# kuailehaha/liuzhou

Measured on AMD Instinct MI355X. Metric: self-play positions/sec (fixed sims/move), higher is better.
Workload: dtype f16

## Files before the change

### include/liuzhou_hip.h

```cpp
#ifndef LIUZHOU_HIP_H
#define LIUZHOU_HIP_H

#include <stdint.h>

#ifdef __cplusplus
extern "C" {
#endif

#if defined(_WIN32)
#define LZ_API
#else
#define LZ_API __attribute__((visibility("default")))
#endif

typedef enum LzStatus {
    LZ_OK = 0,
    LZ_ERR_ARG = -1,
    LZ_ERR_UNSUPPORTED = -2,
    LZ_ERR_LAUNCH = -3,
    LZ_ERR_ALIGN = -4,
    LZ_ERR_ILLEGAL = -5
} LzStatus;


// ... 359 lines not shown

LZ_API int lz_policy_value_loss_fwd_bwd(const float* log_p1, const float* log_p2, const float* log_pmc,
                                        const float* value_logits, const uint8_t* legal_mask,
                                        const float* policy_target, const float* value_target,
                                        const float* soft_value_target, int64_t batch, float soft_label_alpha,
                                        float anti_draw_penalty, float policy_draw_weight,
                                        const float* policy_weight_sum, float grad_scale, float* terms,
                                        float* grad_log_p1, float* grad_log_p2, float* grad_log_pmc,
                                        float* grad_value_logits, void* stream);


#define LZ_TRAJECTORY_RECORD_BYTES 360
LZ_API int lz_pack_trajectory_rows(const float* state_tensors, const uint8_t* legal_masks,
                                   const float* policy_targets, const float* value_targets,
                                   const float* soft_value_targets, int64_t rows, void* records,
                                   int32_t* not_representable, void* stream);
LZ_API int lz_unpack_trajectory_rows(const void* records, int64_t rows, float* state_tensors, uint8_t* legal_masks,
                                     float* policy_targets, float* value_targets, float* soft_value_targets,
                                     void* stream);


LZ_API int lz_symmetry_tables(int32_t* cells, int32_t* actions, int32_t* inverse, int32_t* compose, int32_t* directions);

LZ_API int lz_symmetry_gather_samples(const float* planes, const uint8_t* masks, const float* policy, int64_t n_src,
                                      const int64_t* idx, const void* sym, int32_t sym_width, float* out_planes,
                                      uint8_t* out_masks, float* out_policy, int64_t m, void* stream);

LZ_API int lz_symmetry_transform_states(const LzStateSoA* in, const void* sym, int32_t sym_width,
                                        const LzStateSoA* out, int64_t batch, void* stream);

LZ_API int lz_symmetry_transform_packed(const int64_t* in , const void* sym, int32_t sym_width,
                                        int64_t* out , int64_t batch, void* stream);

#ifdef __cplusplus
}
#endif
#endif
```

### liuzhou_amd/build.py

```python
from __future__ import annotations

import os
import shutil
import subprocess

PKG = os.path.dirname(os.path.abspath(__file__))
CSRC = os.path.join(PKG, "csrc")
LIB = os.path.join(PKG, "libliuzhou_hip.so")
SOURCES = ("lz_ops.hip", "lz_engine.hip", "lz_net.hip", "lz_net_f32.hip", "lz_train.hip", "lz_search.hip", "lz_symmetry.hip")
HEADERS = ("lz_rules.h", "lz_soa.h", "lz_symmetry.h", "lz_wave.h", "lz_rng.h", "lz_net_dev.h", "lz_tree_dev.h", os.path.join("..", "..", "include", "liuzhou_hip.h"))


def hipcc_path() -> str:
    for cand in (os.environ.get("HIPCC"), "/opt/rocm/bin/hipcc", shutil.which("hipcc")):
        if cand and os.path.exists(cand):
            return cand
    raise RuntimeError("hipcc not found (expected /opt/rocm/bin/hipcc)")


HOST_LIB = os.path.join(PKG, "libliuzhou_host.so")
HOST_SOURCE = os.path.join(CSRC, "lz_host.cpp")
HOST_SOURCES = (HOST_SOURCE, os.path.join(CSRC, "lz_scalar.cpp"),
                os.path.join(CSRC, "lz_symmetry_host.cpp"))


def build_host(force: bool = False, verbose: bool = False) -> str:
    deps = list(HOST_SOURCES) + [os.path.join(CSRC, h) for h in HEADERS] + [os.path.join(PKG, "..", "include", "liuzhou_scalar.h")]
    if not force and os.path.exists(HOST_LIB) and all(
            (not os.path.exists(d)) or os.path.getmtime(d) <= os.path.getmtime(HOST_LIB) for d in deps):
        return HOST_LIB
    cxx = os.environ.get("CXX") or shutil.which("g++") or shutil.which("c++")
    if not cxx:
        raise RuntimeError("no host C++ compiler (g++) found for libliuzhou_host.so")
    cmd = [cxx, "-O2", "-std=c++17", "-ffp-contract=off", "-fPIC", "-shared", "-fvisibility=hidden", "-o", HOST_LIB,
           *HOST_SOURCES]
    if verbose:
        print(" ".join(cmd))
    subprocess.check_call(cmd)
    return HOST_LIB


def needs_build() -> bool:
    if not os.path.exists(LIB):
# ... 76 lines not shown
```

### liuzhou_amd/csrc/lz_engine.hip

```cpp
#include <hip/hip_runtime.h>
#include <hip/amd_detail/amd_hip_unsafe_atomics.h>
#include <math.h>
#include <stdint.h>

#include <mutex>

#include "lz_rng.h"
#include "lz_tree_dev.h"

namespace {

__global__ __launch_bounds__(kBlock) void pack_states_kernel(LzStateSoA s, int64_t B, Packed* __restrict__ out) {
    const int64_t i = (int64_t)blockIdx.x * kBlock + threadIdx.x;
    if (i >= B) return;
    State st;
    st.black = cells_equal(s.board + i * 36, 1);
    st.white = cells_equal(s.board + i * 36, -1);
    st.mb = cells_nonzero(s.marks_black + i * 36);
    st.mw = cells_nonzero(s.marks_white + i * 36);
    st.phase = (int)s.phase[i]; st.player = (int)s.current_player[i];
    st.pm_req = (int)s.pending_marks_required[i]; st.pm_rem = (int)s.pending_marks_remaining[i];
    st.pc_req = (int)s.pending_captures_required[i]; st.pc_rem = (int)s.pending_captures_remaining[i];
    st.forced = (int)s.forced_removals_done[i]; st.move_count = (int)s.move_count[i];
    st.msc = (int)s.moves_since_capture[i];
// ... 1434 lines not shown
    const int64_t rn = next_sims + 1;
    if (rn > d->node_cap) return LZ_ERR_ARG;
    if ((int64_t)d->chunk_cap * (d->edge_chunk - (kMaxChildren - 1)) < (int64_t)d->node_cap * kMaxChildren) return LZ_ERR_ARG;
    const bool big = words > kMarkWordsMax;
    const int wpb = big ? 1 : kWavesPerBlock;
    const size_t lds = (size_t)wpb * (words * (sizeof(uint64_t) + sizeof(int)) + 3 * kWave * sizeof(int));
    if (big) {
        static std::mutex mu;
        static bool configured[64] = {};
        int dev = 0;
        if (hipGetDevice(&dev) != hipSuccess || dev < 0 || dev >= 64) return LZ_ERR_LAUNCH;
        std::lock_guard<std::mutex> lk(mu);
        if (!configured[dev]) {
            const size_t most = (size_t)kMarkWordsBig * (sizeof(uint64_t) + sizeof(int)) + 3 * kWave * sizeof(int);
            if (hipFuncSetAttribute(reinterpret_cast<const void*>(tree_advance_kernel<1>),
                                    hipFuncAttributeMaxDynamicSharedMemorySize, (int)most) != hipSuccess) {
                (void)hipGetLastError();
                return LZ_ERR_LAUNCH;
            }
            configured[dev] = true;
        }
    }
    (void)lz_prof_aux_begin(1, stream);
    if (big)
        hipLaunchKernelGGL(tree_advance_kernel<1>, dim3((unsigned)d->num_games), dim3(kWave), lds, as_stream(stream), make_tree(d),
                           played_action, reset, (int)rn, words, dropped, pruned, g_advance_ticks);
    else
        hipLaunchKernelGGL(tree_advance_kernel<kWavesPerBlock>, dim3(gw(d->num_games)), dim3(kBlock), lds, as_stream(stream),
                           make_tree(d), played_action, reset, (int)rn, words, dropped, pruned, g_advance_ticks);
    (void)lz_prof_aux_end(1, stream, d->num_games);
    return st();
}

extern "C++" template <bool CAP, bool FORCED, bool GUMBEL = false>
static int tree_search_launch(const LzTreeDesc* d, const Tree& t, const CapArrays& cap, const ForcedArgs& fa, const GumbelArgs& ga, const LzNetDesc* net, int64_t sims, float* lp1,
                              float* lp2, float* lpmc, float* values, const float* noise, int64_t noise_stride,
                              float epsilon, void* stream) {
    const int64_t B = d->num_games;
    int rc = LZ_OK;
    if (t.live_count != nullptr) {
        if (d->live_count_cap < sims + 2) return LZ_ERR_ARG;
        hipLaunchKernelGGL(tree_live_scan_kernel, dim3(1), dim3(kScanBlock), 0, as_stream(stream), t, t.live_count);
        for (int64_t s = 0; s <= sims; ++s) {
            rc = lz_net_forward_packed_counted_f16(net, d->live_state, B, d->live_count + s, lp1, lp2, lpmc, nullptr, values,
                                                   stream);
            if (rc) return rc;
            if (s == sims) {
                if (s == 0)
                    hipLaunchKernelGGL((tree_expand_kernel<true, true, CAP>), dim3(gw(t.B)), dim3(kBlock), 0, as_stream(stream), t,
                                       lp1, lp2, lpmc, (const float*)nullptr, values, noise, (int)noise_stride, epsilon, (int)s, cap);
                else
                    hipLaunchKernelGGL((tree_expand_kernel<false, true, CAP>), dim3(gw(t.B)), dim3(kBlock), 0, as_stream(stream), t,
                                       lp1, lp2, lpmc, (const float*)nullptr, values, (const float*)nullptr, 0, 0.f, (int)s, cap);
            } else if (s == 0) {
                hipLaunchKernelGGL((tree_expand_select_kernel<true, true, CAP, FORCED, GUMBEL>), dim3(gw(t.B)), dim3(kBlock), 0, as_stream(stream),
                                   t, lp1, lp2, lpmc, values, noise, (int)noise_stride, epsilon, (int)s, cap, fa, ga);
            } else {
                (void)lz_prof_aux_begin(0, stream);
                if (split_step(t.B))
                    hipLaunchKernelGGL((tree_expand_select_split_kernel<true, CAP, FORCED, GUMBEL>), dim3(gw2(t.B)), dim3(kBlock), 0,
                                       as_stream(stream), t, lp1, lp2, lpmc, values, (int)s, cap, fa, ga);
                else
                    hipLaunchKernelGGL((tree_expand_select_kernel<false, true, CAP, FORCED, GUMBEL>), dim3(gw(t.B)), dim3(kBlock), 0, as_stream(stream),
                                       t, lp1, lp2, lpmc, values, nullptr, 0, 0.f, (int)s, cap, fa, ga);
                (void)lz_prof_aux_end(0, stream, B);
            }
            if (s < sims)
                hipLaunchKernelGGL(tree_live_scan_kernel, dim3(1), dim3(kScanBlock), 0, as_stream(stream), t,
                                   t.live_count + (s + 1));
        }
        if (GUMBEL && sims == 0)
            hipLaunchKernelGGL(gumbel_root_kernel, dim3(gw(t.B)), dim3(kBlock), 0, as_stream(stream), t, ga, cap.root_noise);
        return st();
    }
    for (int64_t s = 0; s <= sims; ++s) {
        rc = lz_net_forward_packed_f16(net, d->leaf_state, B, lp1, lp2, lpmc, nullptr, values, stream);
        if (rc) return rc;
        if (s == sims) {
            if (s == 0)
                hipLaunchKernelGGL((tree_expand_kernel<true, false, CAP>), dim3(gw(t.B)), dim3(kBlock), 0, as_stream(stream), t, lp1, lp2,
                                   lpmc, (const float*)nullptr, values, noise, (int)noise_stride, epsilon, (int)s, cap);
            else
                hipLaunchKernelGGL((tree_expand_kernel<false, false, CAP>), dim3(gw(t.B)), dim3(kBlock), 0, as_stream(stream), t, lp1, lp2,
                                   lpmc, (const float*)nullptr, values, (const float*)nullptr, 0, 0.f, (int)s, cap);
        } else if (s == 0) {
            hipLaunchKernelGGL((tree_expand_select_kernel<true, false, CAP, FORCED, GUMBEL>), dim3(gw(t.B)), dim3(kBlock), 0, as_stream(stream), t, lp1,
                               lp2, lpmc, values, noise, (int)noise_stride, epsilon, (int)s, cap, fa, ga);
        } else {
            (void)lz_prof_aux_begin(0, stream);
            if (split_step(t.B))
                hipLaunchKernelGGL((tree_expand_select_split_kernel<false, CAP, FORCED, GUMBEL>), dim3(gw2(t.B)), dim3(kBlock), 0, as_stream(stream),
                                   t, lp1, lp2, lpmc, values, (int)s, cap, fa, ga);
            else
                hipLaunchKernelGGL((tree_expand_select_kernel<false, false, CAP, FORCED, GUMBEL>), dim3(gw(t.B)), dim3(kBlock), 0, as_stream(stream), t, lp1,
                                   lp2, lpmc, values, nullptr, 0, 0.f, (int)s, cap, fa, ga);
            (void)lz_prof_aux_end(0, stream, B);
        }
    }
    if (GUMBEL && sims == 0)
        hipLaunchKernelGGL(gumbel_root_kernel, dim3(gw(t.B)), dim3(kBlock), 0, as_stream(stream), t, ga, cap.root_noise);
    return st();
}

static int tree_search_impl(const LzTreeDesc* d, const LzNetDesc* net, int64_t sims, float* planes, float* lp1,
                            float* lp2, float* lpmc, float* values, const float* noise, int64_t noise_stride,
                            float epsilon, bool continue_trees, void* stream) {
    if (!tree_ok(d) || !net || sims < 0 || !lp1 || !lp2 || !lpmc || !values) return LZ_ERR_ARG;
    if (const int grc = gumbel_check(d)) return grc;
    const int64_t B = d->num_games;
// ... 260 lines not shown
```

### liuzhou_amd/csrc/lz_net.hip

```cpp
#include <hip/hip_runtime.h>
#include <algorithm>
#include <utility>
#include <vector>
#include <math.h>
#include <stdint.h>
#include <stdlib.h>

#include "../../include/liuzhou_hip.h"
#include "lz_net_dev.h"

namespace {

template <int C, int S, int W>
__global__ __launch_bounds__(W * 64, (C == 128 && W == 4) ? 1 : 2) void net_forward_kernel(NetParams P, const float* __restrict__ planes,
                                                            const uint64_t* __restrict__ packed,
                                                            int64_t N, float* __restrict__ lp1,
                                                            float* __restrict__ lp2, float* __restrict__ lpm,
                                                            float* __restrict__ vlogits, float* __restrict__ value) {
    if (P.n_dev != nullptr) { const long long nd = *P.n_dev; N = nd < N ? nd : N; }
    extern __shared__ __attribute__((aligned(16))) unsigned char lds[];
    NetCtx<C, S, W> ctx;
#ifdef LZ_EXP_HEAD_STAMPS
    ctx.t_entry = __builtin_readcyclecounter();
#endif
    net_setup<C, S, W>(P, lds, ctx);
#ifdef LZ_EXP_HEAD_STAMPS
    asm volatile("s_waitcnt vmcnt(0) lgkmcnt(0)" ::: "memory");
    ctx.t_setup = __builtin_readcyclecounter();
#endif
    const uint64_t dbg_t0 = P.debug_stop == 99 ? __builtin_readcyclecounter() : 0;
    const uint64_t dbg_w0 = P.debug_stop == 99 ? wall_clock64() : 0;
    const int64_t n_pass = (N + S - 1) / S;
    for (int64_t pass = blockIdx.x; pass < n_pass; pass += gridDim.x) {
        const int64_t n0 = pass * S;
        const int nvalid = (int)((N - n0) < S ? (N - n0) : S);
        net_pass<C, S, W>(P, lds, ctx, planes, packed, n0, nvalid, lp1, lp2, lpm, vlogits, value);
    }
    if (P.debug_stop == 99 && blockIdx.x == 7 && threadIdx.x == 0) {
        const uint64_t dt = __builtin_readcyclecounter() - dbg_t0, dw = wall_clock64() - dbg_w0;
        value[0] = (float)dt; value[1] = (float)dw;
    }
}
// ... 30 lines not shown
    int cur = -1;
    const float* fp = nullptr;
    for (int pass = blockIdx.x; pass < n_pass; pass += gridDim.x) {
        const int n0 = pass * S;
        int k = 0;
        for (int j = 1; j < num_nets; ++j)
            if (((seg_off[j] + 15) & ~15LL) <= n0) k = j;
        k = __builtin_amdgcn_readfirstlane(k);
        const long long b = (seg_off[k] + 15) & ~15LL, e = seg_off[k + 1] < last ? seg_off[k + 1] : last;
        const int nvalid = (int)((e - n0) < S ? (e - n0) : S);
        if (n0 < b || nvalid <= 0) continue;
        if (k != cur) {
            fp = M.fp[k];
            net_use_weights<C, S, W>(P, ctx, M.wfrag[k], fp);
            cur = k;
        }
        net_pass<C, S, W>(P, lds, ctx, nullptr, packed, (int64_t)n0, nvalid, lp1, lp2, lpm, vlogits, value, fp);
    }
}

template <int C, int S, int W>
int launch_net_multi(const NetParams& P, const MultiNets& M, int num_nets, const uint64_t* packed, int64_t capacity,
                     const int64_t* seg_off, float* lp1, float* lp2, float* lpm, float* vlogits, float* value,
                     int max_blocks, hipStream_t st) {
    using K = Cfg<C, S, W>;
    const int64_t n_pass = (capacity + S - 1) / S;
    int grid = (int)(n_pass < max_blocks ? n_pass : max_blocks);
    if (grid < 1) grid = 1;
    hipLaunchKernelGGL((net_forward_multi_kernel<C, S, W>), dim3(grid), dim3(K::THREADS), K::LDS_BYTES, st, P, M, num_nets,
                       packed, capacity, reinterpret_cast<const long long*>(seg_off), lp1, lp2, lpm, vlogits, value);
    return hipGetLastError() == hipSuccess ? LZ_OK : LZ_ERR_LAUNCH;
}

template <int C, int S, int W>
int configure_net_multi() {
    return hipFuncSetAttribute(reinterpret_cast<const void*>(net_forward_multi_kernel<C, S, W>),
                               hipFuncAttributeMaxDynamicSharedMemorySize, Cfg<C, S, W>::LDS_BYTES) == hipSuccess
               ? LZ_OK : LZ_ERR_LAUNCH;
}

template <int C, int S, int W>
int configure_net() {
    return hipFuncSetAttribute(reinterpret_cast<const void*>(net_forward_kernel<C, S, W>),
                               hipFuncAttributeMaxDynamicSharedMemorySize, Cfg<C, S, W>::LDS_BYTES) == hipSuccess
               ? LZ_OK : LZ_ERR_LAUNCH;
}

}

namespace {
struct NetProf {
    bool on = false;
    int used = 0;
    static constexpr int kMax = 8192;
    hipEvent_t ev[2 * kMax];
    bool created = false;
    double flops = 0.0;
    int64_t evals = 0;
} g_prof;
}

extern "C" void lz_prof_aux_reset(void);

extern "C" {

int lz_prof_enable(int on) {
// ... 78 lines not shown
                if (hipEventCreate(&g_aux.ev[k][i]) != hipSuccess) return LZ_ERR_LAUNCH;
        g_aux.created = true;
    }
    if (g_aux.used[kind] >= AuxProf::kMax) return LZ_OK;
    return hipEventRecord(g_aux.ev[kind][2 * g_aux.used[kind]], reinterpret_cast<hipStream_t>(stream)) == hipSuccess ? LZ_OK : LZ_ERR_LAUNCH;
}
int lz_prof_aux_end(int kind, void* stream, int64_t units) {
    if (!g_prof.on || !g_aux.created || kind < 0 || kind >= AuxProf::kKinds || g_aux.used[kind] >= AuxProf::kMax) return LZ_OK;
    (void)hipEventRecord(g_aux.ev[kind][2 * g_aux.used[kind] + 1], reinterpret_cast<hipStream_t>(stream));
    g_aux.used[kind] += 1; g_aux.units[kind] += units;
    return LZ_OK;
}
int lz_prof_aux_summary(int kind, double* total_ms, int64_t* launches, int64_t* units) {
    if (kind < 0 || kind >= AuxProf::kKinds) return LZ_ERR_ARG;
    double t = 0.0;
    for (int i = 0; i < g_aux.used[kind]; ++i) {
        float ms = 0.f;
        if (hipEventElapsedTime(&ms, g_aux.ev[kind][2 * i], g_aux.ev[kind][2 * i + 1]) != hipSuccess) return LZ_ERR_LAUNCH;
        t += ms;
    }
    if (total_ms) *total_ms = t;
    if (launches) *launches = g_aux.used[kind];
    if (units) *units = g_aux.units[kind];
    return LZ_OK;
}

int64_t lz_net_desc_bytes(void) { return (int64_t)sizeof(LzNetDesc); }

int lz_net_configure(void) {
    const int a = configure_net<64, 16, 8>(), b = configure_net<128, 8, 8>(), c = configure_net<64, 8, 4>(),
              e = configure_net<128, 8, 4>();
    const int ma = configure_net_multi<64, 16, 8>(), mb = configure_net_multi<128, 8, 8>(),
              mc = configure_net_multi<64, 8, 4>(), me = configure_net_multi<128, 8, 4>();
    for (int rc : {a, b, c, e, ma, mb, mc, me})
        if (rc != LZ_OK) return rc;
    return LZ_OK;
}

int lz_net_forward_f32_dispatch(const LzNetDesc* d, const float* planes, const uint64_t* packed, int64_t N, float* lp1,
                                float* lp2, float* lpmc, float* value_logits, float* value, const int64_t* n_dev,
                                void* stream);

static int net_forward_impl(const LzNetDesc* d, const float* planes, const uint64_t* packed, int64_t N, float* lp1,
                            float* lp2, float* lpmc, float* value_logits, float* value, void* stream,
                            const int64_t* n_dev = nullptr) {
    if (!d || N < 0) return LZ_ERR_ARG;
    if (N == 0) return LZ_OK;
    if (!d->wfrag || !d->fparams || (!planes && !packed)) return LZ_ERR_ARG;
    const bool heads = lp1 && lp2 && lpmc;
    if (!heads && (lp1 || lp2 || lpmc || !value)) return LZ_ERR_ARG;
    if (d->blocks < 0 || d->blocks > (LZ_NET_MAX_LAYERS - 2) / 2 || d->num_layers != 2 + 2 * d->blocks) return LZ_ERR_ARG;
    if ((reinterpret_cast<uintptr_t>(d->wfrag) & 15) || (reinterpret_cast<uintptr_t>(d->fparams) & 15)) return LZ_ERR_ALIGN;
    if (d->flags & (4 | 8))
        return lz_net_forward_f32_dispatch(d, planes, packed, N, lp1, lp2, lpmc, value_logits, value, n_dev, stream);
    NetParams P = make_net_params(d);
#ifdef LZ_EXP_SAME_LAYER
    for (int i = 3; i < 1 + 2 * d->blocks; ++i) P.layer_off[i] = d->layer_offsets[1 + ((i - 1) & 1)];
#endif
    P.n_dev = reinterpret_cast<const long long*>(n_dev);
    P.debug_stop = getenv("LZ_NET_DEBUG_STOP") ? atoi(getenv("LZ_NET_DEBUG_STOP")) : 0;
    const bool half_wg = d->channels == 64 && (d->flags & 1);
    const int max_blocks = d->max_blocks > 0 ? d->max_blocks : (half_wg ? 512 : 256);
    hipStream_t st = reinterpret_cast<hipStream_t>(stream);
    if (d->channels != 64 && d->channels != 128) return LZ_ERR_UNSUPPORTED;
    const bool prof = g_prof.on && g_prof.used < NetProf::kMax;
    if (prof) (void)hipEventRecord(g_prof.ev[2 * g_prof.used], st);
    const bool wide = d->channels == 128 && (d->flags & 2);
    const int rc = d->channels == 64
                       ? (half_wg
                              ? launch_net<64, 8, 4>(P, planes, packed, N, lp1, lp2, lpmc, value_logits, value, max_blocks, st)
                              : launch_net<64, 16, 8>(P, planes, packed, N, lp1, lp2, lpmc, value_logits, value, max_blocks, st))
                       : (wide ? launch_net<128, 8, 4>(P, planes, packed, N, lp1, lp2, lpmc, value_logits, value, max_blocks, st)
                               : launch_net<128, 8, 8>(P, planes, packed, N, lp1, lp2, lpmc, value_logits, value, max_blocks, st));
    if (prof) { (void)hipEventRecord(g_prof.ev[2 * g_prof.used + 1], st); g_prof.used += 1; g_prof.evals += N; }
    return rc;
}

int lz_net_forward_f16(const LzNetDesc* d, const float* planes, int64_t N, float* lp1, float* lp2, float* lpmc,
                       float* value_logits, float* value, void* stream) {
    return net_forward_impl(d, planes, nullptr, N, lp1, lp2, lpmc, value_logits, value, stream);
}

int lz_net_forward_packed_f16(const LzNetDesc* d, const void* packed_states, int64_t N, float* lp1, float* lp2,
                              float* lpmc, float* value_logits, float* value, void* stream) {
    return net_forward_impl(d, nullptr, reinterpret_cast<const uint64_t*>(packed_states), N, lp1, lp2, lpmc,
                            value_logits, value, stream);
}

int lz_net_forward_packed_counted_f16(const LzNetDesc* d, const void* packed_states, int64_t capacity,
                                      const int64_t* count, float* lp1, float* lp2, float* lpmc, float* value_logits,
                                      float* value, void* stream) {
    if (!count) return LZ_ERR_ARG;
    return net_forward_impl(d, nullptr, reinterpret_cast<const uint64_t*>(packed_states), capacity, lp1, lp2, lpmc,
                            value_logits, value, stream, count);
}

static int multi_net_check(const LzNetDesc* a, const LzNetDesc* b) {
    if (a->channels != b->channels || a->blocks != b->blocks || a->num_layers != b->num_layers ||
        a->max_blocks != b->max_blocks || a->wfrag_bytes != b->wfrag_bytes || a->fparams_bytes != b->fparams_bytes ||
        (a->flags & 3) != (b->flags & 3))
        return LZ_ERR_ARG;
    for (int i = 0; i < LZ_NET_MAX_LAYERS; ++i)
        if (i < a->num_layers && a->layer_offsets[i] != b->layer_offsets[i]) return LZ_ERR_ARG;
    for (int i = 0; i < 4; ++i)
        if (a->head_frag_offsets[i] != b->head_frag_offsets[i]) return LZ_ERR_ARG;
    const int32_t oa[13] = {a->off_stem_bias, a->off_block0, a->off_trunk_a, a->off_trunk_b, a->off_head_bias, a->off_p_gwT,
                            a->off_p_a2, a->off_p_b2, a->off_p_out, a->off_v_w1T, a->off_v_b1, a->off_v_w2T, a->off_v_b2};
    const int32_t ob[13] = {b->off_stem_bias, b->off_block0, b->off_trunk_a, b->off_trunk_b, b->off_head_bias, b->off_p_gwT,
                            b->off_p_a2, b->off_p_b2, b->off_p_out, b->off_v_w1T, b->off_v_b1, b->off_v_w2T, b->off_v_b2};
    for (int i = 0; i < 13; ++i)
        if (oa[i] != ob[i]) return LZ_ERR_ARG;
    return LZ_OK;
}

int lz_net_multi_validate(const LzNetDesc* const* nets, int num_nets) {
    if (!nets || num_nets < 1 || num_nets > kMaxNets) return LZ_ERR_ARG;
    for (int k = 0; k < num_nets; ++k) {
        const LzNetDesc* n = nets[k];
        if (!n || !n->wfrag || !n->fparams) return LZ_ERR_ARG;
        if (n->flags & (4 | 8)) return LZ_ERR_UNSUPPORTED;
        if ((reinterpret_cast<uintptr_t>(n->wfrag) & 15) || (reinterpret_cast<uintptr_t>(n->fparams) & 15)) return LZ_ERR_ALIGN;
    }
    const LzNetDesc* d = nets[0];
    if (d->blocks < 0 || d->blocks > (LZ_NET_MAX_LAYERS - 2) / 2 || d->num_layers != 2 + 2 * d->blocks) return LZ_ERR_ARG;
    for (int k = 1; k < num_nets; ++k) {
        const int rc = multi_net_check(d, nets[k]);
        if (rc) return rc;
    }
    return d->channels == 64 || d->channels == 128 ? LZ_OK : LZ_ERR_UNSUPPORTED;
// ... 38 lines not shown
```

### liuzhou_amd/csrc/lz_net_dev.h

```cpp
#pragma once
#include <hip/hip_runtime.h>
#include <math.h>
#include <stdint.h>

#include "../../include/liuzhou_hip.h"
#include "lz_wave.h"

namespace {


typedef _Float16 h8 __attribute__((ext_vector_type(8)));
typedef _Float16 h4 __attribute__((ext_vector_type(4)));
typedef float f4 __attribute__((ext_vector_type(4)));
typedef unsigned int u4 __attribute__((ext_vector_type(4)));

struct Rsrc { __amdgpu_buffer_rsrc_t w, f; };
__device__ __forceinline__ __amdgpu_buffer_rsrc_t make_rsrc(const void* p, int bytes) {
    return __builtin_amdgcn_make_buffer_rsrc(const_cast<void*>(p), 0, bytes, 0x00020000);
}
__device__ __forceinline__ h8 load_wfrag(__amdgpu_buffer_rsrc_t r, int lane_off, int byte_off) {
    return __builtin_bit_cast(h8, __builtin_amdgcn_raw_buffer_load_b128(r, lane_off, byte_off, 0));
}
__device__ __forceinline__ f4 load_f4(__amdgpu_buffer_rsrc_t r, int lane_float_off, int float_off) {
    return __builtin_bit_cast(f4, __builtin_amdgcn_raw_buffer_load_b128(r, lane_float_off * 4, float_off * 4, 0));
// ... 418 lines not shown
    using K = Cfg<C, S, W>;
    static_assert(K::CT == K::CG * K::CTW && (K::CTW == 2 || K::CTW == 4), "each wave owns 2 or 4 output-channel tiles");
    static_assert(K::NT % 9 == 0 && K::PG * K::CG == K::WAVES, "waves = cell groups x channel groups");
    static_assert(S * 32 <= K::THREADS, "global pooling uses 2 lanes per (sample, 4-channel group)");
    constexpr int NTHR = K::THREADS;
    const int tid = threadIdx.x;
    const int lane = tid & 63;
    const int wave = __builtin_amdgcn_readfirstlane(tid >> 6);
    const int pg = wave % K::PG, cg = wave / K::PG;
    const int tile0 = pg * 9;
    ctx.tid = tid; ctx.lane = lane; ctx.wave = wave; ctx.pg = pg; ctx.cg = cg;
    ctx.ct0 = cg * K::CTW;
    ctx.chan0 = ctx.ct0 * 16;
    ctx.rw = make_rsrc(P.wfrag, P.wfrag_bytes);
    ctx.rf = make_rsrc(P.fp, P.fparams_bytes);
#pragma unroll
    for (int i = 0; i < 9; ++i) {
        const int n = tile_cell_calc(pg, i, lane & 15);
        ctx.base[i] = K::ACT_OFF + board_row(n) * K::STRIDE + (lane >> 4) * 32 - K::STRIDE;
    }
    ctx.mirror = (pg & 1) != 0;
    ctx.row_step = ctx.mirror ? -7 * K::STRIDE : 7 * K::STRIDE;
    for (int i = tid; i < K::ZERO_OFF / 16; i += NTHR) reinterpret_cast<uint4*>(lds + K::ACT_OFF)[i] = make_uint4(0, 0, 0, 0);
    for (int i = tid; i < (K::PAR_OFF - K::POOL_OFF) / 4; i += NTHR) reinterpret_cast<uint32_t*>(lds + K::POOL_OFF)[i] = 0u;
}

template <int C, int S, int W>
__device__ __forceinline__ void net_use_weights(const NetParams& P, NetCtx<C, S, W>& ctx, const _Float16* wfrag,
                                                const float* fp) {
    ctx.rw = make_rsrc(wfrag, P.wfrag_bytes);
    ctx.rf = make_rsrc(fp, P.fparams_bytes);
}

template <int C, int S, int W>
__device__ __forceinline__ void net_pass(const NetParams& P, unsigned char* lds, NetCtx<C, S, W>& ctx, const float* planes,
                                         const uint64_t* packed, int64_t n0, int nvalid, float* lp1, float* lp2,
                                         float* lpm, float* vlogits, float* value, const float* fp_net = nullptr) {
    using K = Cfg<C, S, W>;
    constexpr int NW = K::CTW;
    using Acc = AccT<NW>;
    constexpr int NTHR = K::THREADS;
    const int tid = ctx.tid, lane = ctx.lane, wave = ctx.wave, cg = ctx.cg, ct0 = ctx.ct0, chan0 = ctx.chan0;
    const float* fp = fp_net != nullptr ? fp_net : P.fp;
    const __amdgpu_buffer_rsrc_t rw = ctx.rw, rf = ctx.rf;
    int (&base)[9] = ctx.base;
    const bool mirror = ctx.mirror;
    const int row_step = ctx.row_step;
    float* gvec = reinterpret_cast<float*>(lds + K::G_OFF);
    float* plog = reinterpret_cast<float*>(lds + K::PLOG_OFF);
    float* par = reinterpret_cast<float*>(lds + K::PAR_OFF);
    int tid_s = tid;
    asm volatile("" : "+v"(tid_s));
    const int st_s = tid_s >> 5, st_p = tid_s & 31;
    uint64_t rec0 = 0, rec1 = 0, rec2 = 0, rec3 = 0;
    if (packed != nullptr && st_s < nvalid) {
        const uint64_t* rec = packed + (n0 + st_s) * 4;
        rec0 = rec[0]; rec1 = rec[1]; rec2 = rec[2]; rec3 = rec[3];
    }
#ifdef LZ_EXP_HEAD_STAMPS
    asm volatile("s_waitcnt vmcnt(0) lgkmcnt(0)" ::: "memory");
    const uint64_t t_before_barrier = __builtin_readcyclecounter();
#endif
    __syncthreads();
#ifdef LZ_EXP_HEAD_STAMPS
    const uint64_t t_after_barrier = __builtin_readcyclecounter();
    uint64_t fst[4] = {0, 0, 0, 0};
#define LZ_FSTAMP(k) { asm volatile("s_waitcnt vmcnt(0) lgkmcnt(0)" ::: "memory"); fst[k] = __builtin_readcyclecounter(); }
#else
#define LZ_FSTAMP(k)
#endif
    LZ_FSTAMP(0)
    if (packed != nullptr) {
        if (st_s < S) {
            const bool on = st_s < nvalid;
            const bool white = (rec0 >> 53) & 1;
            const int phase = on ? (int)((rec0 >> 50) & 7) : 0;
            const uint64_t own = white ? rec1 : rec0, opp = white ? rec0 : rec1;
            const uint64_t sm = white ? rec3 : rec2, om = white ? rec2 : rec3;
            for (int p = st_p; p < 36; p += 32) {
                _Float16 row[32];
#pragma unroll
                for (int k = 0; k < 32; ++k) row[k] = (_Float16)0.f;
                if (on) {
                    row[0] = (_Float16)(float)((own >> p) & 1);
                    row[1] = (_Float16)(float)((opp >> p) & 1);
                    row[2] = (_Float16)(float)((sm >> p) & 1);
                    row[3] = (_Float16)(float)((om >> p) & 1);
#pragma unroll
                    for (int ph = 1; ph <= 7; ++ph) row[3 + ph] = (_Float16)(phase == ph ? 1.f : 0.f);
// ... 180 lines not shown
                d = __builtin_amdgcn_mfma_f32_16x16x32_f16(kb == 0 ? wo0 : wo1, b, d, 0, 0, 0);
            }
            if (lane_h < 16) {
                plog[(s * 3 + 0) * 36 + p] = d[0];
                plog[(s * 3 + 1) * 36 + p] = d[1];
                plog[(s * 3 + 2) * 36 + p] = d[2];
            }
        }
    }
    __syncthreads();
    LZ_HSTAMP(5)
    {
        constexpr int ROWS = S * 3, PASSES = (ROWS + 4 * K::WAVES - 1) / (4 * K::WAVES);
        const int k4 = lane_h & 15;
#pragma unroll
        for (int pass = 0; pass < PASSES; ++pass) {
            const int row = (pass * K::WAVES + wave) * 4 + (lane_h >> 4);
            const bool on = k4 < 9 && row < ROWS;
            const f4 v = on ? *reinterpret_cast<const f4*>(plog + row * 36 + 4 * k4) : (f4){-INFINITY, -INFINITY, -INFINITY, -INFINITY};
            float mx = fmaxf(fmaxf(v[0], v[1]), fmaxf(v[2], v[3]));
            mx = fmaxf(mx, lzw::dpp_f32<0x128, 0xf>(mx, mx));
            mx = fmaxf(mx, lzw::dpp_f32<0x124, 0xf>(mx, mx));
            mx = fmaxf(mx, lzw::dpp_f32<0x122, 0xf>(mx, mx));
            mx = fmaxf(mx, lzw::dpp_f32<0x121, 0xf>(mx, mx));
            float e = 0.f;
            if (on) e = ((expf(v[0] - mx) + expf(v[1] - mx)) + expf(v[2] - mx)) + expf(v[3] - mx);
            e += lzw::dpp_f32<0x128, 0xf>(e, e);
            e += lzw::dpp_f32<0x124, 0xf>(e, e);
            e += lzw::dpp_f32<0x122, 0xf>(e, e);
            e += lzw::dpp_f32<0x121, 0xf>(e, e);
            const int s = row / 3, h = row - s * 3;
            if (on && s < nvalid) {
                const float lse = mx + logf(e);
                float* dst = (h == 0 ? lp1 : h == 1 ? lp2 : lpm) + (n0 + s) * 36 + 4 * k4;
                dst[0] = v[0] - lse; dst[1] = v[1] - lse; dst[2] = v[2] - lse; dst[3] = v[3] - lse;
            }
        }
    }
    __syncthreads();
    LZ_HSTAMP(6)
    }
    if (P.debug_stop == 5) { if (lane_h == 0 && x[0][0][0] == 123.f) lp1[0] = 1.f; return; }
    if (K::HP == 2) store_head<C, S, NW>(x, lds, base, ht1 - 4, rf, P.head_bias + kHead, lane);
    else if (ht0 >= 4) store_head<C, S, NW>(acc, lds, base, ht0 - 4, rf, P.head_bias + kHead, lane);
    constexpr int R1 = (8 + K::WAVES - 1) / K::WAVES, R2 = (7 + K::WAVES - 1) / K::WAVES;
    h8 w1[R1][6], w2[R2][4];
    f4 b1[R1], b2[R2];
#pragma unroll
    for (int r = 0; r < R1; ++r) {
        const int ct = wave + r * K::WAVES < 8 ? wave + r * K::WAVES : 7;
        fc_load<8, 6>(rw, P.hf_w1, ct, lane_h, w1[r]);
        b1[r] = load_f4(rf, (lane_h >> 4) * 4, P.v_b1 + ct * 16);
    }
#pragma unroll
    for (int r = 0; r < R2; ++r) {
        const int ct = wave + r * K::WAVES < 7 ? wave + r * K::WAVES : 6;
        fc_load<7, 4>(rw, P.hf_w2, ct, lane_h, w2[r]);
        b2[r] = load_f4(rf, (lane_h >> 4) * 4, P.v_b2 + ct * 16);
    }
    __syncthreads();
    LZ_HSTAMP(7)
    gpool64<C, S>(lds, tid_h);
    __syncthreads();
    LZ_HSTAMP(8)
#pragma unroll
    for (int r = 0; r < R1; ++r) {
        const int ct = wave + r * K::WAVES;
// ... 16 lines not shown
#pragma unroll
            for (int q = 0; q < 4; ++q)
                if (o + q < kBins) vl[s * K::VL_STRIDE + o + q] = d[q] + b2[r][q];
        }
    }
    __syncthreads();
    LZ_HSTAMP(10)
    {
        constexpr int SPW = (S + K::WAVES - 1) / K::WAVES;
        float v0[SPW], v1[SPW], mx[SPW], e0[SPW], e1[SPW], sum[SPW], ex[SPW];
#pragma unroll
        for (int i = 0; i < SPW; ++i) {
            const int s = wave + i * K::WAVES;
            const bool on = s < nvalid;
            v0[i] = on ? vl[s * K::VL_STRIDE + lane_h] : 0.f;
            v1[i] = (on && lane_h + 64 < kBins) ? vl[s * K::VL_STRIDE + lane_h + 64] : -INFINITY;
        }
#pragma unroll
        for (int i = 0; i < SPW; ++i) mx[i] = lzw::wave_max(fmaxf(v0[i], v1[i]));
#pragma unroll
        for (int i = 0; i < SPW; ++i) {
            e0[i] = expf(v0[i] - mx[i]);
            e1[i] = lane_h + 64 < kBins ? expf(v1[i] - mx[i]) : 0.f;
        }
#pragma unroll
        for (int i = 0; i < SPW; ++i) sum[i] = lzw::wave_sum(e0[i] + e1[i]);
#pragma unroll
        for (int i = 0; i < SPW; ++i)
            ex[i] = lzw::wave_sum(e0[i] * (-1.0f + 0.02f * (float)lane_h) + e1[i] * (-1.0f + 0.02f * (float)(lane_h + 64)));
#pragma unroll
        for (int i = 0; i < SPW; ++i) {
            const int s = wave + i * K::WAVES;
            if (s < nvalid) {
                if (lane_h == 0 && value != nullptr) value[n0 + s] = ex[i] / sum[i];
                if (vlogits != nullptr) {
                    vlogits[(n0 + s) * kBins + lane_h] = v0[i];
                    if (lane_h + 64 < kBins) vlogits[(n0 + s) * kBins + lane_h + 64] = v1[i];
                }
            }
        }
    }
#ifdef LZ_EXP_HEAD_STAMPS
    LZ_HSTAMP(11)
    __syncthreads();
    if (blockIdx.x == 0 && lane_h == 0 && vlogits != nullptr) {
        for (int k = 0; k < 12; ++k) vlogits[wave * 24 + k] = (float)(hstamps[k] - hstamps[0]);
        vlogits[wave * 24 + 12] = (float)(ctx.t_setup - ctx.t_entry);
        vlogits[wave * 24 + 13] = (float)(fst[0] - ctx.t_setup);
        vlogits[wave * 24 + 14] = (float)(fst[1] - fst[0]);
        vlogits[wave * 24 + 15] = (float)(fst[2] - fst[1]);
        vlogits[wave * 24 + 16] = (float)(fst[3] - fst[2]);
        vlogits[wave * 24 + 17] = (float)(hstamps[0] - fst[3]);
        vlogits[wave * 24 + 18] = (float)(t_before_barrier - ctx.t_setup);
        vlogits[wave * 24 + 19] = (float)(t_after_barrier - t_before_barrier);
        vlogits[wave * 24 + 20] = (float)(ctx.t_entry & 0xFFFFFF);
    }
#endif
}

inline NetParams make_net_params(const LzNetDesc* d) {
    NetParams P;
    P.wfrag = reinterpret_cast<const _Float16*>(d->wfrag);
    P.fp = d->fparams;
    for (int i = 0; i < LZ_NET_MAX_LAYERS; ++i) P.layer_off[i] = i < d->num_layers ? d->layer_offsets[i] : 0;
    P.blocks = d->blocks;
    P.n_dev = nullptr;
    P.wfrag_bytes = (int)d->wfrag_bytes; P.fparams_bytes = (int)d->fparams_bytes;
    P.debug_stop = 0;
    P.hf_gw = d->head_frag_offsets[0]; P.hf_w1 = d->head_frag_offsets[1]; P.hf_w2 = d->head_frag_offsets[2];
    P.hf_out = d->head_frag_offsets[3];
// ... 8 lines not shown
```

Measured before the change: 12380.

## Fuse live-leaf compaction into net forward via in-kernel gather of live games

Adds a gather variant of the f16 net forward kernel. Each block ballots leaf_kind into live masks in LDS, builds a prefix popcount, maps compacted rows to game indices, and evaluates only live leaves, writing outputs back at the original slots. The tree search uses it when the batch would exceed one pass per block and no split step applies. This replaces the separate live scan plus full-batch evaluation, at the price of redundant mask and prefix work in every block and extra LDS use.

Measured after the change: 12690, median of 6. 1.02x the previous value.

```diff
diff --git a/include/liuzhou_hip.h b/include/liuzhou_hip.h
--- a/include/liuzhou_hip.h
+++ b/include/liuzhou_hip.h
@@ -415,6 +415,10 @@
 LZ_API int lz_symmetry_transform_packed(const int64_t* in , const void* sym, int32_t sym_width,
                                         int64_t* out , int64_t batch, void* stream);
 
+LZ_API int lz_net_forward_packed_gather_f16(const LzNetDesc* net, const void* packed_states, const int32_t* leaf_kind,
+                                            int64_t num_slots, int64_t* count_out, float* log_p1, float* log_p2,
+                                            float* log_pmc, float* value_logits, float* value, void* stream);
+
 #ifdef __cplusplus
 }
 #endif
diff --git a/liuzhou_amd/build.py b/liuzhou_amd/build.py
--- a/liuzhou_amd/build.py
+++ b/liuzhou_amd/build.py
@@ -8,7 +8,7 @@
 CSRC = os.path.join(PKG, "csrc")
 LIB = os.path.join(PKG, "libliuzhou_hip.so")
 SOURCES = ("lz_ops.hip", "lz_engine.hip", "lz_net.hip", "lz_net_f32.hip", "lz_train.hip", "lz_search.hip", "lz_symmetry.hip")
-HEADERS = ("lz_rules.h", "lz_soa.h", "lz_symmetry.h", "lz_wave.h", "lz_rng.h", "lz_net_dev.h", "lz_tree_dev.h", os.path.join("..", "..", "include", "liuzhou_hip.h"))
+HEADERS = ("lz_rules.h", "lz_soa.h", "lz_symmetry.h", "lz_wave.h", "lz_rng.h", "lz_net_dev.h", "lz_live_index.h", "lz_tree_dev.h", os.path.join("..", "..", "include", "liuzhou_hip.h"))
 
 
 def hipcc_path() -> str:
diff --git a/liuzhou_amd/csrc/lz_engine.hip b/liuzhou_amd/csrc/lz_engine.hip
--- a/liuzhou_amd/csrc/lz_engine.hip
+++ b/liuzhou_amd/csrc/lz_engine.hip
@@ -1490,14 +1490,28 @@
     return st();
 }
 
+int lz_net_gather_supported(const LzNetDesc* d, int64_t num_slots);
+void lz_net_launch_shape(const LzNetDesc* d, int* max_blocks, int* samples);
+
+static bool tree_gather_path(const LzNetDesc* net, int64_t B) {
+    const char* e = getenv("LZ_TREE_GATHER");
+    if (e && e[0] == '0') return false;
+    if (!lz_net_gather_supported(net, B)) return false;
+    if (e && e[0] == '1') return true;
+    int max_blocks = 0, samples = 1;
+    lz_net_launch_shape(net, &max_blocks, &samples);
+    return (B + samples - 1) / samples > max_blocks && !split_step(B);
+}
+
 extern "C++" template <bool CAP, bool FORCED, bool GUMBEL = false>
 static int tree_search_launch(const LzTreeDesc* d, const Tree& t, const CapArrays& cap, const ForcedArgs& fa, const GumbelArgs& ga, const LzNetDesc* net, int64_t sims, float* lp1,
                               float* lp2, float* lpmc, float* values, const float* noise, int64_t noise_stride,
                               float epsilon, void* stream) {
     const int64_t B = d->num_games;
     int rc = LZ_OK;
-    if (t.live_count != nullptr) {
-        if (d->live_count_cap < sims + 2) return LZ_ERR_ARG;
+    if (t.live_count != nullptr && d->live_count_cap < sims + 2) return LZ_ERR_ARG;
+    const bool gather = t.live_count != nullptr && tree_gather_path(net, B);
+    if (t.live_count != nullptr && !gather) {
         hipLaunchKernelGGL(tree_live_scan_kernel, dim3(1), dim3(kScanBlock), 0, as_stream(stream), t, t.live_count);
         for (int64_t s = 0; s <= sims; ++s) {
             rc = lz_net_forward_packed_counted_f16(net, d->live_state, B, d->live_count + s, lp1, lp2, lpmc, nullptr, values,
@@ -1532,7 +1546,9 @@
         return st();
     }
     for (int64_t s = 0; s <= sims; ++s) {
-        rc = lz_net_forward_packed_f16(net, d->leaf_state, B, lp1, lp2, lpmc, nullptr, values, stream);
+        rc = gather ? lz_net_forward_packed_gather_f16(net, d->leaf_state, t.leaf_kind, B, d->live_count + s, lp1, lp2, lpmc,
+                                                       nullptr, values, stream)
+                    : lz_net_forward_packed_f16(net, d->leaf_state, B, lp1, lp2, lpmc, nullptr, values, stream);
         if (rc) return rc;
         if (s == sims) {
             if (s == 0)
diff --git a/liuzhou_amd/csrc/lz_live_index.h b/liuzhou_amd/csrc/lz_live_index.h
--- /dev/null
+++ b/liuzhou_amd/csrc/lz_live_index.h
@@ -0,0 +1,53 @@
+#pragma once
+#include <stdint.h>
+
+#if defined(__HIPCC__) || defined(__CUDACC__)
+#define LZ_LIVE_HD __host__ __device__
+#else
+#define LZ_LIVE_HD
+#endif
+
+namespace lzlive {
+
+LZ_LIVE_HD inline int popc64(uint64_t m) {
+#if defined(__HIP_DEVICE_COMPILE__)
+    return __popcll(m);
+#else
+    return __builtin_popcountll(m);
+#endif
+}
+
+LZ_LIVE_HD inline int mask_words(int64_t games) { return (int)((games + 63) >> 6); }
+
+LZ_LIVE_HD inline int prefix_popcounts(const uint64_t* masks, int words, int* prefix) {
+    int run = 0;
+    for (int w = 0; w < words; ++w) { prefix[w] = run; run += popc64(masks[w]); }
+    return run;
+}
+
+LZ_LIVE_HD inline int find_word(const int* prefix, int words, int row) {
+    int lo = 0, hi = words - 1;
+    while (lo < hi) {
+        const int mid = (lo + hi + 1) >> 1;
+        if (prefix[mid] <= row) lo = mid; else hi = mid - 1;
+    }
+    return lo;
+}
+
+LZ_LIVE_HD inline int select_bit(uint64_t m, int k) {
+    int pos = 0;
+#pragma unroll
+    for (int width = 32; width >= 1; width >>= 1) {
+        const uint64_t low = m & ((1ull << width) - 1ull);
+        const int c = popc64(low);
+        if (k >= c) { k -= c; m >>= width; pos += width; }
+    }
+    return pos;
+}
+
+LZ_LIVE_HD inline int row_to_game(const uint64_t* masks, const int* prefix, int words, int row) {
+    const int w = find_word(prefix, words, row);
+    return w * 64 + select_bit(masks[w], row - prefix[w]);
+}
+
+}
diff --git a/liuzhou_amd/csrc/lz_net.hip b/liuzhou_amd/csrc/lz_net.hip
--- a/liuzhou_amd/csrc/lz_net.hip
+++ b/liuzhou_amd/csrc/lz_net.hip
@@ -8,6 +8,7 @@
 
 #include "../../include/liuzhou_hip.h"
 #include "lz_net_dev.h"
+#include "lz_live_index.h"
 
 namespace {
 
@@ -104,6 +105,105 @@
     return hipGetLastError() == hipSuccess ? LZ_OK : LZ_ERR_LAUNCH;
 }
 
+constexpr int kLiveKind = 1;
+constexpr int kGatherUnroll = 8;
+template <int S> constexpr int gather_head_bytes() { return ((2 * S + 1) * 4 + 15) & ~15; }
+template <int C, int S, int W> constexpr int gather_lds_limit() { return (C == 64 && W == 4) ? 80 * 1024 : 160 * 1024; }
+template <int C, int S, int W>
+int64_t gather_lds_bytes(int64_t B) {
+    const int64_t words = (B + 63) >> 6;
+    return Cfg<C, S, W>::LDS_BYTES + gather_head_bytes<S>() + words * 12;
+}
+
+template <int C, int S, int W>
+__global__ __launch_bounds__(W * 64, (C == 128 && W == 4) ? 1 : 2) void net_forward_gather_kernel(
+        NetParams P, const uint64_t* __restrict__ packed, const int* __restrict__ leaf_kind, int B,
+        unsigned long long* __restrict__ count_out, int even_rounds, float* __restrict__ lp1, float* __restrict__ lp2,
+        float* __restrict__ lpm, float* __restrict__ vlogits, float* __restrict__ value) {
+    using K = Cfg<C, S, W>;
+    extern __shared__ __attribute__((aligned(16))) unsigned char lds[];
+    NetCtx<C, S, W> ctx;
+    net_setup<C, S, W>(P, lds, ctx);
+    const int words = (B + 63) >> 6;
+    int* tab = reinterpret_cast<int*>(lds + K::LDS_BYTES);
+    uint64_t* masks = reinterpret_cast<uint64_t*>(lds + K::LDS_BYTES + gather_head_bytes<S>());
+    int* prefix = reinterpret_cast<int*>(masks + words);
+    const int tid = ctx.tid, lane = ctx.lane, wave = ctx.wave;
+    const int rounds = (B + K::THREADS - 1) / K::THREADS;
+    for (int r0 = 0; r0 < rounds; r0 += kGatherUnroll) {
+        int kind[kGatherUnroll];
+#pragma unroll
+        for (int u = 0; u < kGatherUnroll; ++u) {
+            const int g = (r0 + u) * K::THREADS + tid;
+            kind[u] = g < B ? leaf_kind[g] : kLiveKind - 1;
+        }
+#pragma unroll
+        for (int u = 0; u < kGatherUnroll; ++u) {
+            const unsigned long long m = __ballot(kind[u] == kLiveKind);
+            const int w = (r0 + u) * W + wave;
+            if (lane == 0 && w < words) masks[w] = m;
+        }
+    }
+    __syncthreads();
+    if (wave == 0) {
+        int run = 0;
+        for (int w0 = 0; w0 < words; w0 += 64) {
+            const int w = w0 + lane;
+            const int c = w < words ? lzlive::popc64(masks[w]) : 0;
+            int incl = c;
+#pragma unroll
+            for (int d = 1; d < 64; d <<= 1) {
+                const int v = __shfl_up(incl, d, 64);
+                if (lane >= d) incl += v;
+            }
+            if (w < words) prefix[w] = run + incl - c;
+            run += __shfl(incl, 63, 64);
+        }
+        if (lane == 0) tab[2 * S] = run;
+    }
+    __syncthreads();
+    const int n = __builtin_amdgcn_readfirstlane(tab[2 * S]);
+    if (blockIdx.x == 0 && tid == 0) *count_out = (unsigned long long)n;
+    const int n_pass = (n + S - 1) / S;
+    int stride = gridDim.x;
+    if (even_rounds && n_pass > 0) {
+        const int r = (n_pass + stride - 1) / stride;
+        stride = (n_pass + r - 1) / r;
+    }
+    if ((int)blockIdx.x >= stride) return;
+    int par = 0;
+    for (int pass = blockIdx.x; pass < n_pass; pass += stride, par ^= 1) {
+        const int n0 = pass * S;
+        const int nvalid = (n - n0) < S ? (n - n0) : S;
+        int* slot_tab = tab + par * S;
+        if (tid < S) slot_tab[tid] = tid < nvalid ? lzlive::row_to_game(masks, prefix, words, n0 + tid) : 0;
+        __syncthreads();
+        net_pass<C, S, W, true>(P, lds, ctx, nullptr, packed, 0, nvalid, lp1, lp2, lpm, vlogits, value, nullptr, slot_tab);
+    }
+}
+
+template <int C, int S, int W>
+int launch_net_gather(const NetParams& P, const uint64_t* packed, const int* leaf_kind, int64_t B,
+                      unsigned long long* count_out, int even_rounds, float* lp1, float* lp2, float* lpm, float* vlogits,
+                      float* value, int max_blocks, hipStream_t st) {
+    using K = Cfg<C, S, W>;
+    const int64_t lds = gather_lds_bytes<C, S, W>(B);
+    if (lds > gather_lds_limit<C, S, W>()) return LZ_ERR_UNSUPPORTED;
+    const int64_t n_pass = (B + S - 1) / S;
+    int grid = (int)(n_pass < max_blocks ? n_pass : max_blocks);
+    if (grid < 1) grid = 1;
+    hipLaunchKernelGGL((net_forward_gather_kernel<C, S, W>), dim3(grid), dim3(K::THREADS), (size_t)lds, st, P, packed,
+                       leaf_kind, (int)B, count_out, even_rounds, lp1, lp2, lpm, vlogits, value);
+    return hipGetLastError() == hipSuccess ? LZ_OK : LZ_ERR_LAUNCH;
+}
+
+template <int C, int S, int W>
+int configure_net_gather() {
+    return hipFuncSetAttribute(reinterpret_cast<const void*>(net_forward_gather_kernel<C, S, W>),
+                               hipFuncAttributeMaxDynamicSharedMemorySize, gather_lds_limit<C, S, W>()) == hipSuccess
+               ? LZ_OK : LZ_ERR_LAUNCH;
+}
+
 template <int C, int S, int W>
 int configure_net_multi() {
     return hipFuncSetAttribute(reinterpret_cast<const void*>(net_forward_multi_kernel<C, S, W>),
@@ -248,7 +348,9 @@
               e = configure_net<128, 8, 4>();
     const int ma = configure_net_multi<64, 16, 8>(), mb = configure_net_multi<128, 8, 8>(),
               mc = configure_net_multi<64, 8, 4>(), me = configure_net_multi<128, 8, 4>();
-    for (int rc : {a, b, c, e, ma, mb, mc, me})
+    const int ga = configure_net_gather<64, 16, 8>(), gb = configure_net_gather<128, 8, 8>(),
+              gc = configure_net_gather<64, 8, 4>(), ge = configure_net_gather<128, 8, 4>();
+    for (int rc : {a, b, c, e, ma, mb, mc, me, ga, gb, gc, ge})
         if (rc != LZ_OK) return rc;
     return LZ_OK;
 }
@@ -311,6 +413,62 @@
                             value_logits, value, stream, count);
 }
 
+static int net_gather_shape(const LzNetDesc* d, int64_t num_slots) {
+    if (d->flags & (4 | 8)) return LZ_ERR_UNSUPPORTED;
+    if (d->channels != 64 && d->channels != 128) return LZ_ERR_UNSUPPORTED;
+    if (num_slots > (int64_t)INT32_MAX - 1024) return LZ_ERR_UNSUPPORTED;
+    const bool half_wg = d->channels == 64 && (d->flags & 1), wide = d->channels == 128 && (d->flags & 2);
+    const int64_t need = d->channels == 64 ? (half_wg ? gather_lds_bytes<64, 8, 4>(num_slots) : gather_lds_bytes<64, 16, 8>(num_slots))
+                                           : (wide ? gather_lds_bytes<128, 8, 4>(num_slots) : gather_lds_bytes<128, 8, 8>(num_slots));
+    const int64_t limit = half_wg ? gather_lds_limit<64, 8, 4>() : gather_lds_limit<128, 8, 8>();
+    return need <= limit ? LZ_OK : LZ_ERR_UNSUPPORTED;
+}
+int lz_net_gather_supported(const LzNetDesc* d, int64_t num_slots) {
+    return d && num_slots > 0 && net_gather_shape(d, num_slots) == LZ_OK;
+}
+void lz_net_launch_shape(const LzNetDesc* d, int* max_blocks, int* samples) {
+    const bool half_wg = d->channels == 64 && (d->flags & 1);
+    *max_blocks = d->max_blocks > 0 ? d->max_blocks : (half_wg ? 512 : 256);
+    *samples = d->channels == 64 && !half_wg ? 16 : 8;
+}
+
+int lz_net_forward_packed_gather_f16(const LzNetDesc* d, const void* packed_states, const int32_t* leaf_kind,
+                                     int64_t num_slots, int64_t* count_out, float* lp1, float* lp2, float* lpmc,
+                                     float* value_logits, float* value, void* stream) {
+    if (!d || num_slots < 0) return LZ_ERR_ARG;
+    if (num_slots == 0) return LZ_OK;
+    if (!d->wfrag || !d->fparams || !packed_states || !leaf_kind || !count_out) return LZ_ERR_ARG;
+    const bool heads = lp1 && lp2 && lpmc;
+    if (!heads && (lp1 || lp2 || lpmc || !value)) return LZ_ERR_ARG;
+    if (d->blocks < 0 || d->blocks > (LZ_NET_MAX_LAYERS - 2) / 2 || d->num_layers != 2 + 2 * d->blocks) return LZ_ERR_ARG;
+    if ((reinterpret_cast<uintptr_t>(d->wfrag) & 15) || (reinterpret_cast<uintptr_t>(d->fparams) & 15)) return LZ_ERR_ALIGN;
+    const int src = net_gather_shape(d, num_slots);
+    if (src) return src;
+    NetParams P = make_net_params(d);
+    P.debug_stop = getenv("LZ_NET_DEBUG_STOP") ? atoi(getenv("LZ_NET_DEBUG_STOP")) : 0;
+    const char* ev = getenv("LZ_NET_EVEN_ROUNDS");
+    const int even_rounds = ev && ev[0] == '0' ? 0 : 1;
+    const bool half_wg = d->channels == 64 && (d->flags & 1);
+    const bool wide = d->channels == 128 && (d->flags & 2);
+    const int max_blocks = d->max_blocks > 0 ? d->max_blocks : (half_wg ? 512 : 256);
+    hipStream_t st = reinterpret_cast<hipStream_t>(stream);
+    const uint64_t* packed = reinterpret_cast<const uint64_t*>(packed_states);
+    unsigned long long* cnt = reinterpret_cast<unsigned long long*>(count_out);
+    const bool prof = g_prof.on && g_prof.used < NetProf::kMax;
+    if (prof) (void)hipEventRecord(g_prof.ev[2 * g_prof.used], st);
+    const int rc = d->channels == 64
+                       ? (half_wg ? launch_net_gather<64, 8, 4>(P, packed, leaf_kind, num_slots, cnt, even_rounds, lp1, lp2, lpmc,
+                                                                value_logits, value, max_blocks, st)
+                                  : launch_net_gather<64, 16, 8>(P, packed, leaf_kind, num_slots, cnt, even_rounds, lp1, lp2, lpmc,
+                                                                 value_logits, value, max_blocks, st))
+                       : (wide ? launch_net_gather<128, 8, 4>(P, packed, leaf_kind, num_slots, cnt, even_rounds, lp1, lp2, lpmc,
+                                                              value_logits, value, max_blocks, st)
+                               : launch_net_gather<128, 8, 8>(P, packed, leaf_kind, num_slots, cnt, even_rounds, lp1, lp2, lpmc,
+                                                              value_logits, value, max_blocks, st));
+    if (prof) { (void)hipEventRecord(g_prof.ev[2 * g_prof.used + 1], st); g_prof.used += 1; g_prof.evals += num_slots; }
+    return rc;
+}
+
 static int multi_net_check(const LzNetDesc* a, const LzNetDesc* b) {
     if (a->channels != b->channels || a->blocks != b->blocks || a->num_layers != b->num_layers ||
         a->max_blocks != b->max_blocks || a->wfrag_bytes != b->wfrag_bytes || a->fparams_bytes != b->fparams_bytes ||
diff --git a/liuzhou_amd/csrc/lz_net_dev.h b/liuzhou_amd/csrc/lz_net_dev.h
--- a/liuzhou_amd/csrc/lz_net_dev.h
+++ b/liuzhou_amd/csrc/lz_net_dev.h
@@ -474,10 +474,11 @@
     ctx.rf = make_rsrc(fp, P.fparams_bytes);
 }
 
-template <int C, int S, int W>
+template <int C, int S, int W, bool GATHER = false>
 __device__ __forceinline__ void net_pass(const NetParams& P, unsigned char* lds, NetCtx<C, S, W>& ctx, const float* planes,
                                          const uint64_t* packed, int64_t n0, int nvalid, float* lp1, float* lp2,
-                                         float* lpm, float* vlogits, float* value, const float* fp_net = nullptr) {
+                                         float* lpm, float* vlogits, float* value, const float* fp_net = nullptr,
+                                         const int* slot_tab = nullptr) {
     using K = Cfg<C, S, W>;
     constexpr int NW = K::CTW;
     using Acc = AccT<NW>;
@@ -496,7 +497,7 @@
     const int st_s = tid_s >> 5, st_p = tid_s & 31;
     uint64_t rec0 = 0, rec1 = 0, rec2 = 0, rec3 = 0;
     if (packed != nullptr && st_s < nvalid) {
-        const uint64_t* rec = packed + (n0 + st_s) * 4;
+        const uint64_t* rec = packed + (GATHER ? (int64_t)slot_tab[st_s] : n0 + st_s) * 4;
         rec0 = rec[0]; rec1 = rec[1]; rec2 = rec[2]; rec3 = rec[3];
     }
 #ifdef LZ_EXP_HEAD_STAMPS
@@ -743,7 +744,7 @@
             const int s = row / 3, h = row - s * 3;
             if (on && s < nvalid) {
                 const float lse = mx + logf(e);
-                float* dst = (h == 0 ? lp1 : h == 1 ? lp2 : lpm) + (n0 + s) * 36 + 4 * k4;
+                float* dst = (h == 0 ? lp1 : h == 1 ? lp2 : lpm) + (GATHER ? (int64_t)slot_tab[s] : n0 + s) * 36 + 4 * k4;
                 dst[0] = v[0] - lse; dst[1] = v[1] - lse; dst[2] = v[2] - lse; dst[3] = v[3] - lse;
             }
         }
@@ -826,10 +827,19 @@
         for (int i = 0; i < SPW; ++i) {
             const int s = wave + i * K::WAVES;
             if (s < nvalid) {
+                if constexpr (GATHER) {
+                    const int64_t r = slot_tab[s];
+                    if (lane_h == 0 && value != nullptr) value[r] = ex[i] / sum[i];
+                    if (vlogits != nullptr) {
+                        vlogits[r * kBins + lane_h] = v0[i];
+                        if (lane_h + 64 < kBins) vlogits[r * kBins + lane_h + 64] = v1[i];
+                    }
+                } else {
                 if (lane_h == 0 && value != nullptr) value[n0 + s] = ex[i] / sum[i];
                 if (vlogits != nullptr) {
                     vlogits[(n0 + s) * kBins + lane_h] = v0[i];
                     if (lane_h + 64 < kBins) vlogits[(n0 + s) * kBins + lane_h + 64] = v1[i];
+                }
                 }
             }
         }
```
